# kausaltech/reina-model

Hardware: NVIDIA B200
Metric: agent-days/sec (HUS 1.7M) (higher is better)
Workload: dtype int32/f32 state, f64 uniforms

## Files before the change

### include/reina_b200.h

```cpp
#ifndef REINA_B200_H
#define REINA_B200_H

#include <stdint.h>

#ifdef __cplusplus
extern "C" {
#endif

#define RB_MAX_AGES 128
#define RB_MAX_VARIANTS 4
#define RB_MAX_ROWS 96
#define RB_NCDF 100
#define RB_MAX_IMPORT_EVENTS 8
#define RB_MAX_VACC 8
#define RB_MAX_IMPORT_CLASSES 16
#define RB_N_PLACES 6
#define RB_IOT_LEN 21

enum { RB_ASYMPTOMATIC = 0, RB_MILD, RB_SEVERE, RB_CRITICAL, RB_FATAL };
enum { RB_SUSCEPTIBLE = 0, RB_INCUBATION, RB_ILLNESS, RB_HOSPITALIZED, RB_IN_ICU, RB_RECOVERED, RB_DEAD };
enum { RB_NO_PROBLEMOS = 0, RB_TOO_MANY_INFECTEES, RB_TOO_MANY_CONTACTS, RB_HOSPITAL_ACCOUNTING_FAILURE,
       RB_NEGATIVE_CONTACTS, RB_MALLOC_FAILURE, RB_OTHER_FAILURE, RB_WRONG_STATE,
       RB_CONTACT_PROBABILITY_FAILURE, RB_INFECTEES_MISMATCH };
enum { RB_NO_TESTING = 0, RB_ALL_WITH_SYMPTOMS_CT, RB_ALL_WITH_SYMPTOMS, RB_ONLY_SEVERE_SYMPTOMS };
// ... 116 lines not shown
int rb_read_queue(rb_engine *e, int32_t replica, int32_t *out, int32_t cap, int32_t *n);
int rb_read_available(rb_engine *e, int32_t replica, int32_t *beds_icu);
float rb_last_step_ms(rb_engine *e);
#define RB_N_KERNELS 5
int rb_step_profiled(rb_engine *e, int32_t n_days, float *ms_per_kernel);
int rb_step_timed(rb_engine *e, int32_t n_days, float *ms_per_kernel, int32_t *launches_per_kernel, float *wall_ms);
int rb_comm_init(rb_engine *e, int32_t rank, int32_t nranks, const uint8_t *unique_id128);
int32_t rb_comm_rank(rb_engine *e);
int32_t rb_comm_size(rb_engine *e);
int rb_comm_allreduce(rb_engine *e, double *inout, int64_t n, int32_t op);
int rb_comm_allgather(rb_engine *e, const void *in, void *out, int64_t bytes_per_rank);
int rb_reduce_moments(rb_engine *e, int32_t day0, int32_t n, double *sum, double *sumsq, int64_t *n_replicas);

int rb_shard_unique_id(uint8_t *out128);
int rb_shard_init(rb_engine *e, int32_t rank, int32_t nranks, const uint8_t *unique_id128, float exchange_capacity);
int rb_shard_init_local(rb_engine **engines, int32_t nranks, float exchange_capacity);
int32_t rb_shard_rank(rb_engine *e);
int32_t rb_shard_nranks(rb_engine *e);
int64_t rb_shard_message_bytes(rb_engine *e);
int32_t rb_shard_exchange(rb_engine *e);

int64_t rb_state_bytes(rb_engine *e);
int rb_save_state(rb_engine *e, void *out, int64_t capacity);
int rb_load_state(rb_engine *e, const void *in, int64_t n_bytes);

int rb_branch(rb_engine *e, const int32_t *src, const uint32_t *seed);
int rb_read_seeds(rb_engine *e, uint32_t *out);

void rb_debug_flag(rb_engine *e, int32_t flag);
int rb_debug_phase_cycles(rb_engine *e, int32_t replica, long long *out16);

int64_t rb_launch_count(rb_engine *e);
int64_t rb_copied_bytes(rb_engine *e, int32_t direction);
const char *rb_last_error(void);

#ifdef __cplusplus
}
#endif
#endif
```

### reina_b200/_abi.py

```python
import ctypes as C
import os

import numpy as np

RB_MAX_AGES = 128
RB_MAX_VARIANTS = 4
RB_MAX_ROWS = 96
RB_NCDF = 100
RB_MAX_IMPORT_EVENTS = 8
RB_MAX_VACC = 8
RB_MAX_IMPORT_CLASSES = 16
RB_N_PLACES = 6
RB_IOT_LEN = 21
RB_N_TABLES = 6
RB_TX_BINS = 65
RB_PLACE_ROOT = RB_N_PLACES

ATTRS = ['susceptible', 'vaccinated', 'infected', 'all_infected', 'detected', 'all_detected',
         'in_icu', 'cum_icu', 'in_ward', 'dead', 'recovered', 'non_hospital_deaths', 'new_infections']
RB_N_ATTRS = len(ATTRS)
SCALARS = ['available_icu_units', 'available_hospital_beds', 'total_icu_units', 'total_hospital_beds',
           'total_infections', 'total_infectors', 'exposed_per_day', 'ct_cases_per_day', 'table_epoch',
           'day']
RB_S_CONTACTS0 = len(SCALARS)
# ... 32 lines not shown
    _fields_ = [
        ('testing_mode', C.c_int32), ('p_detected_anyway', C.c_float),
        ('p_successful_tracing', C.c_float), ('beds_delta', C.c_int32), ('icu_delta', C.c_int32),
        ('table_epoch', C.c_int32), ('n_imports', C.c_int32),
        ('import_amount', C.c_int32 * RB_MAX_IMPORT_EVENTS),
        ('import_variant', C.c_int32 * RB_MAX_IMPORT_EVENTS),
        ('trickle', C.c_int32 * RB_MAX_VARIANTS), ('n_vacc', C.c_int32),
        ('vacc_nr', C.c_int32 * RB_MAX_VACC), ('vacc_min_age', C.c_int32 * RB_MAX_VACC),
        ('vacc_max_age', C.c_int32 * RB_MAX_VACC), ('vacc_slot', C.c_int32 * RB_MAX_VACC),
        ('import_traced', C.c_int32), ('reserved', C.c_int32 * 3),
    ]


AGENT_DTYPE = np.dtype([
    ('infector', '<i4'), ('n_infected', '<i4'), ('days_left', '<i2'), ('day_of_illness', '<i2'),
    ('day_of_vaccination', '<i2'), ('state', 'u1'), ('severity', 'u1'), ('variant', 'u1'),
    ('flags', 'u1'), ('ward_days', 'u1'), ('icu_days', 'u1')], align=True)
assert AGENT_DTYPE.itemsize == 20, AGENT_DTYPE.itemsize

_HERE = os.path.dirname(os.path.abspath(__file__))
CUDA_LIB_PATH = os.environ.get('REINA_B200_LIB') or os.path.join(_HERE, 'libreina_b200.so')

SYMBOLS = ['create', 'destroy', 'reset', 'set_initial_state', 'step_profiled', 'set_contact_table', 'set_schedule', 'step', 'sync', 'day',
           'snapshot', 'row_len', 'read_stats', 'read_moments', 'read_per_age', 'problem', 'sample', 'read_agents',
           'read_queue', 'read_available', 'last_step_ms', 'launch_count', 'last_error', 'rng_block']


TX_SYMBOLS = ['transmission_len', 'transmission_stats', 'read_infection_days']
SX_SYMBOLS = ['transmission_settings_len', 'transmission_settings', 'read_infection_places']
BRANCH_SYMBOLS = ['branch', 'read_seeds']
SHARD_SYMBOLS = ['shard_unique_id', 'shard_init', 'shard_init_local', 'shard_rank', 'shard_nranks', 'shard_message_bytes', 'shard_exchange',
                 'state_bytes', 'save_state', 'load_state',
                 'comm_init', 'comm_rank', 'comm_size', 'comm_allreduce', 'comm_allgather', 'reduce_moments',
                 'step_timed', 'debug_flag', 'debug_phase_cycles', 'copied_bytes'] + TX_SYMBOLS + SX_SYMBOLS + BRANCH_SYMBOLS
SH_SHIFT = 12


def owner_of(agent_index, nranks):
    return (np.asarray(agent_index) >> SH_SHIFT) % nranks


class EngineError(RuntimeError):
    pass


def _ptr(a, ctype):
    return a.ctypes.data_as(C.POINTER(ctype))


class Library:

    def __init__(self, path, prefix):
        if not os.path.exists(path):
            raise EngineError(
                '%s not found: build it with `python -c "import __graft_entry__ as g; g.build()"` '
                '(there is no CPU fallback)' % path)
        self.path, self.prefix = path, prefix
        self.dll = C.CDLL(path)
        f = {}
        for name in SYMBOLS:
            f[name] = getattr(self.dll, prefix + name)
        vp = C.c_void_p
        f['create'].argtypes = [C.POINTER(Config), C.POINTER(C.c_int32), C.POINTER(C.c_int32),
                                C.POINTER(Variant), C.POINTER(C.c_int32), C.POINTER(C.c_int32),
                                C.POINTER(C.c_float), C.POINTER(vp)]
        f['destroy'].argtypes = [vp]
        f['destroy'].restype = None
# ... 24 lines not shown
        f['last_step_ms'].argtypes = [vp]
        f['last_step_ms'].restype = C.c_float
        f['launch_count'].argtypes = [vp]
        f['launch_count'].restype = C.c_int64
        f['last_error'].argtypes = []
        f['last_error'].restype = C.c_char_p
        if prefix == 'rb_':
            for name in SHARD_SYMBOLS:
                f[name] = getattr(self.dll, prefix + name)
            f['shard_unique_id'].argtypes = [C.c_char_p]
            f['shard_init'].argtypes = [vp, C.c_int32, C.c_int32, C.c_char_p, C.c_float]
            f['shard_init_local'].argtypes = [C.POINTER(vp), C.c_int32, C.c_float]
            f['shard_rank'].argtypes = [vp]
            f['shard_nranks'].argtypes = [vp]
            f['shard_message_bytes'].argtypes = [vp]
            f['shard_message_bytes'].restype = C.c_int64
            f['shard_exchange'].argtypes = [vp]
            f['state_bytes'].argtypes = [vp]
            f['state_bytes'].restype = C.c_int64
            f['save_state'].argtypes = [vp, C.c_void_p, C.c_int64]
            f['load_state'].argtypes = [vp, C.c_void_p, C.c_int64]
            f['comm_init'].argtypes = [vp, C.c_int32, C.c_int32, C.c_char_p]
            f['comm_rank'].argtypes = [vp]
            f['comm_size'].argtypes = [vp]
            f['comm_allreduce'].argtypes = [vp, C.POINTER(C.c_double), C.c_int64, C.c_int32]
            f['comm_allgather'].argtypes = [vp, C.c_void_p, C.c_void_p, C.c_int64]
            f['reduce_moments'].argtypes = [vp, C.c_int32, C.c_int32, C.POINTER(C.c_double), C.POINTER(C.c_double), C.POINTER(C.c_int64)]
            f['step_timed'].argtypes = [vp, C.c_int32, C.POINTER(C.c_float), C.POINTER(C.c_int32), C.POINTER(C.c_float)]
            f['debug_flag'].argtypes = [vp, C.c_int32]
            f['debug_flag'].restype = None
            f['debug_phase_cycles'].argtypes = [vp, C.c_int32, C.c_void_p]
            f['copied_bytes'].argtypes = [vp, C.c_int32]
            f['copied_bytes'].restype = C.c_int64
        self.f = f
        if prefix == 'rb_':
            self.bind_transmission()
            self.bind_settings()
            self.bind_branch()

    def bind_transmission(self):
        f, vp = self.f, C.c_void_p
        for name in TX_SYMBOLS:
            f[name] = getattr(self.dll, self.prefix + name)
        f['transmission_len'].argtypes = [vp]
        f['transmission_len'].restype = C.c_int32
        f['transmission_stats'].argtypes = [vp, C.POINTER(C.c_int32)]
        f['read_infection_days'].argtypes = [vp, C.c_int32, C.POINTER(C.c_int32)]

    def bind_settings(self):
        f, vp = self.f, C.c_void_p
        for name in SX_SYMBOLS:
            f[name] = getattr(self.dll, self.prefix + name)
        f['transmission_settings_len'].argtypes = [vp]
        f['transmission_settings_len'].restype = C.c_int32
        f['transmission_settings'].argtypes = [vp, C.POINTER(C.c_int32), C.c_int32, C.POINTER(C.c_int32)]
        f['read_infection_places'].argtypes = [vp, C.c_int32, C.POINTER(C.c_int32), C.c_int32, C.POINTER(C.c_int32)]

    def bind_branch(self):
        f, vp = self.f, C.c_void_p
        for name in BRANCH_SYMBOLS:
            f[name] = getattr(self.dll, self.prefix + name)
        f['branch'].argtypes = [vp, C.POINTER(C.c_int32), C.POINTER(C.c_uint32)]
        f['read_seeds'].argtypes = [vp, C.POINTER(C.c_uint32)]

    def check(self, rc, what):
        if rc != 0:
# ... 194 lines not shown
        out = np.empty((self.n_replicas, self.lib.f['transmission_settings_len'](self.h)), dtype=np.int32)
        self.lib.check(self.lib.f['transmission_settings'](self.h, _ptr(ep, C.c_int32), ep.size, _ptr(out, C.c_int32)),
                       'transmission_settings')
        return out

    def read_infection_places(self, replica, epoch_of_day):
        ep = np.ascontiguousarray(epoch_of_day, dtype=np.int32)
        out = np.empty(self.n_agents, dtype=np.int32)
        self.lib.check(self.lib.f['read_infection_places'](self.h, replica, _ptr(ep, C.c_int32), ep.size, _ptr(out, C.c_int32)),
                       'read_infection_places')
        return out

    def branch(self, src, seeds):
        s = np.ascontiguousarray(src, dtype=np.int32)
        k = np.ascontiguousarray(seeds, dtype=np.uint32)
        assert s.shape == k.shape == (self.n_replicas,)
        self.lib.check(self.lib.f['branch'](self.h, _ptr(s, C.c_int32), _ptr(k, C.c_uint32)), 'branch')

    def read_seeds(self):
        out = np.empty((self.n_replicas, self.cfg.max_days + 1), dtype=np.uint32)
        self.lib.check(self.lib.f['read_seeds'](self.h, _ptr(out, C.c_uint32)), 'read_seeds')
        return out

    def last_step_ms(self):
        return float(self.lib.f['last_step_ms'](self.h))

    def launch_count(self):
        return int(self.lib.f['launch_count'](self.h))

    def copied_bytes(self):
        f = self.lib.f['copied_bytes']
        return int(f(self.h, 0)), int(f(self.h, 1))


def shard_init_local(engines, exchange_capacity=0.0):
    lib = engines[0].lib
    arr = (C.c_void_p * len(engines))(*[e.h for e in engines])
    try:
        lib.check(lib.f['shard_init_local'](arr, len(engines), exchange_capacity), 'shard_init_local')
    except EngineError:
        for e in engines:
            e.half_joined = True
        raise
    for k, e in enumerate(engines):
        e.rank, e.nranks = k, len(engines)


def shard_unique_id(lib=None):
    lib = lib or cuda_library()
    buf = C.create_string_buffer(128)
    lib.check(lib.f['shard_unique_id'](buf), 'shard_unique_id')
    return buf.raw
```

### reina_b200/csrc/branch.cuh

```cuda
#ifndef REINA_B200_BRANCH_CUH
#define REINA_B200_BRANCH_CUH

#include "state.cuh"

__device__ __forceinline__ void branch_copy_bytes(void *dst, const void *src, size_t bytes, size_t tid, size_t nt) {
    if ((((uintptr_t)dst | (uintptr_t)src | bytes) & 15u) == 0) {
        uint4 *d = (uint4 *)dst; const uint4 *s = (const uint4 *)src;
        for (size_t i = tid; i < bytes / 16; i += nt) d[i] = s[i];
    } else {
        uint32_t *d = (uint32_t *)dst; const uint32_t *s = (const uint32_t *)src;
        for (size_t i = tid; i < bytes / 4; i += nt) d[i] = s[i];
    }
}

__global__ void k_branch_copy(Eng G, uint32_t *seed_of_day, const int32_t *src, const uint32_t *seed, int today) {
    const int j = blockIdx.y, s = src[j];
    const size_t tid = (size_t)blockIdx.x * blockDim.x + threadIdx.x, nt = (size_t)gridDim.x * blockDim.x;
    const size_t M = (size_t)G.max_days + 1;
    if (s != j) {
        const size_t N = G.Npad, W = G.sus_words, Q = 2 * (size_t)G.cap_queue, S = M * G.row_len;
        branch_copy_bytes(G.hot + j * N, G.hot + s * N, N * sizeof(uint32_t), tid, nt);
        branch_copy_bytes(G.rec + j * N, G.rec + s * N, N * sizeof(AgentRec), tid, nt);
        branch_copy_bytes(G.sus + j * W, G.sus + s * W, W * sizeof(uint32_t), tid, nt);
        branch_copy_bytes(G.det + j * W, G.det + s * W, W * sizeof(uint32_t), tid, nt);
        branch_copy_bytes(G.q_key + j * Q, G.q_key + s * Q, Q * sizeof(unsigned long long), tid, nt);
        branch_copy_bytes(G.q_agent + j * Q, G.q_agent + s * Q, Q * sizeof(int32_t), tid, nt);
        branch_copy_bytes(G.stats + j * S, G.stats + s * S, S * sizeof(int32_t), tid, nt);
        for (size_t i = tid; i < 2 * (size_t)G.n_seg; i += nt) G.seg_n[2 * (size_t)G.n_seg * j + i] = make_uint2(0u, 0u);
    }
    if (blockIdx.x != 0) return;
    const uint32_t *cs = reinterpret_cast<const uint32_t *>(&G.ctr[s]);
    uint32_t *cd = reinterpret_cast<uint32_t *>(&G.ctr[j]);
    const uint32_t seed_word = (uint32_t)(offsetof(RepCtr, seed) / 4);
    if (s != j)
        for (uint32_t w = threadIdx.x; w < (uint32_t)(sizeof(RepCtr) / 4); w += blockDim.x) cd[w] = w == seed_word ? seed[j] : cs[w];
    else if (threadIdx.x == 0) cd[seed_word] = seed[j];
    const uint32_t *hs = seed_of_day + (size_t)s * M;
    uint32_t *hd = seed_of_day + (size_t)j * M;
    for (size_t d = threadIdx.x; d < M; d += blockDim.x)
        if ((int)d >= today) hd[d] = seed[j]; else if (s != j) hd[d] = hs[d];
}

__global__ void k_branch_rebuild(Eng G, const int32_t *src) {
    const int r = blockIdx.y;
    if (src[r] == r) return;
    RepCtr *c = &G.ctr[r];
    const size_t base = (size_t)r * G.Npad;
    const uint32_t cur = c->lsel;
    for (int a = blockIdx.x * blockDim.x + threadIdx.x; a < G.N; a += gridDim.x * blockDim.x) {
        uint32_t h = G.hot[base + a];
        const uint32_t st = H_STATE(h);
        if (st == RB_SUSCEPTIBLE) continue;
        G.perm[base + a] = sweep_slot(G, c, (uint32_t)a);
        if (!((st >= RB_INCUBATION && st <= RB_IN_ICU) || (st >= RB_RECOVERED && !(h & H_INCL)))) continue;
        if (h & H_QUEUED) h |= H_DET;
        list_add(G, r, c, cur, (uint32_t)a, h);
    }
}

__global__ void k_init_seeds(Eng G, uint32_t *seed_of_day, uint32_t seed, int from_ctr) {
    const int r = blockIdx.x;
// ... 6 lines not shown
```

### reina_b200/csrc/engine.cu

```cuda
#include "state.cuh"
#include "boundary.cuh"
#include "sweep.cuh"
#include "contacts.cuh"
#include "shard.cuh"
#include "setup.cuh"
#include "run.cuh"
#include "transmission.cuh"
#include "branch.cuh"

static thread_local char g_err[512];
#define CK(call) do { cudaError_t e_ = (call); if (e_ != cudaSuccess) { snprintf(g_err, sizeof g_err, "%s:%d %s: %s", __FILE__, __LINE__, #call, cudaGetErrorString(e_)); return 1; } } while (0)

#define MAX_GROUPS 8
struct ReplicaGroup {
    int r0, R;
    int sweep_blocks, list_blocks, resolve_blocks;
    cudaStream_t stream;
    cudaEvent_t ev_stagger, ev_join;
    cudaGraphExec_t graph[2];
};

struct rb_engine {
    rb_config cfg;
    Eng G;
// ... 173 lines not shown
    float cc = cfg->contact_capacity > 0 ? cfg->contact_capacity : 1.0f;
    G.cap_items = pow2_at_least((uint64_t)((double)N * cc) + 4096);
    G.cap_succ = pow2_at_least((uint64_t)N / 8 + 4096);
    G.cap_events = pow2_at_least((uint64_t)N / 16 + 2048);
    G.cap_queue = pow2_at_least((uint64_t)N / 8 + 2048);
    const size_t RN = (size_t)R * G.Npad;
    cudaDeviceProp prop; CK(cudaGetDeviceProperties(&prop, cfg->device));
    const int sms = prop.multiProcessorCount;
    e->run_ctas = 0; e->run_boundary_ctas = 1;
    {
        int per_sm = 0;
        CK(cudaOccupancyMaxActiveBlocksPerMultiprocessor(&per_sm, k_run, RUN_THREADS, 0));
        const long long total = (long long)per_sm * sms;
        bool on = false;
        if (const char *s = getenv("RB_PERSISTENT")) on = atoi(s) != 0;
        if (on && total >= 2LL * R) {
            long long t = total / R; if (t > 64) t = 64;
            if (const char *s = getenv("RB_RUN_CTAS")) { const int v = atoi(s); if (v >= 1 && (long long)v * R <= total) t = v; }
            e->run_ctas = (int)t;
            int b = 1; while (b * 2 <= t && b * 2 <= 16) b *= 2;
            e->run_boundary_ctas = b;
        }
    }
    {
        int ng, pct;
        group_config(R, &ng, &pct);
        long long ctas = (long long)sms * SW_CTAS_PER_SM * (ng > 1 ? pct : 100) / 100 / ((R + ng - 1) / ng);
        if (ctas < 1) ctas = 1;
        long long S = 2 * ctas * SW_WARPS, most = (long long)N / 256;
        if (e->run_ctas) S = 2LL * e->run_ctas * RUN_WARPS;
        if (S > most) S = most;
        G.n_seg = (uint32_t)(S < 1 ? 1 : S);
        G.seg_cap = ((uint32_t)N + G.n_seg - 1) / G.n_seg;
    }
    G.sus_words = ((G.Npad + 31) / 32 + 32 + 3) & ~3;
    if (dalloc(e, &G.hot, RN) || dalloc(e, &G.perm, RN) || dalloc(e, &G.rec, RN) ||
        dalloc(e, &G.sus, (size_t)R * G.sus_words) || dalloc(e, &G.det, (size_t)R * G.sus_words) || dalloc(e, &G.alist, (size_t)R * 2 * G.n_seg * G.seg_cap) || dalloc(e, &G.seg_n, (size_t)R * 2 * G.n_seg) || dalloc(e, &G.items, (size_t)R * G.cap_items) || dalloc(e, &G.succ, (size_t)R * G.cap_succ) ||
        dalloc(e, &G.ev_key, (size_t)R * G.cap_events) || dalloc(e, &G.ev_agent, (size_t)R * G.cap_events) ||
        dalloc(e, &G.q_key, (size_t)R * 2 * G.cap_queue) || dalloc(e, &G.q_agent, (size_t)R * 2 * G.cap_queue) ||
        dalloc(e, &G.ctr, (size_t)R) || dalloc(e, &G.stats, (size_t)R * (cfg->max_days + 1) * G.row_len) ||
        dalloc(e, &e->seed_of_day, (size_t)R * (cfg->max_days + 1)) ||
        dalloc(e, &e->d_sched, (size_t)cfg->max_days + 1) ||
        dalloc(e, &e->d_moments, 2 * ((size_t)cfg->max_days + 1) * G.row_len + 2)) { rb_destroy(e); return 1; }
    G.sched = e->d_sched;
    e->h_sched.assign(cfg->max_days + 1, rb_day_params());
    e->n_table_slots = 1024;
    if (dalloc(e, &e->d_tables, (size_t)e->n_table_slots)) { rb_destroy(e); return 1; }
    CK(cudaMemset(e->d_tables, 0, sizeof(DevTable *) * e->n_table_slots));
    G.tables = e->d_tables;
    e->tables.assign(e->n_table_slots, nullptr);
    rb_variant *dv; int32_t *d_as, *d_ga, *d_ilo, *d_ihi; float *d_icum; uint8_t *d_ab;
    if (dalloc(e, &dv, (size_t)cfg->n_variants) || dalloc(e, &d_as, (size_t)cfg->n_ages + 1) || dalloc(e, &d_ga, (size_t)cfg->n_ages) ||
        dalloc(e, &d_ilo, (size_t)RB_MAX_IMPORT_CLASSES) || dalloc(e, &d_ihi, (size_t)RB_MAX_IMPORT_CLASSES) ||
        dalloc(e, &d_icum, (size_t)RB_MAX_IMPORT_CLASSES) || dalloc(e, &d_ab, (size_t)(G.Npad >> 10) + 2)) { rb_destroy(e); return 1; }
    {
        std::vector<uint8_t> ab((size_t)(G.Npad >> 10) + 2);
        int age = 0;
        for (size_t b = 0; b < ab.size(); b++) {
            int64_t a = (int64_t)b << 10; if (a > N - 1) a = N - 1;
            while (age < cfg->n_ages - 1 && e->age_start[age + 1] <= a) age++;
            ab[b] = (uint8_t)age;
        }
        CK(cudaMemcpy(d_ab, ab.data(), ab.size(), cudaMemcpyHostToDevice));
    }
    e->h_variants.assign(variants, variants + cfg->n_variants);
    CK(cudaMemcpy(dv, variants, sizeof(rb_variant) * cfg->n_variants, cudaMemcpyHostToDevice));
    CK(cudaMemcpy(d_as, e->age_start.data(), sizeof(int32_t) * (cfg->n_ages + 1), cudaMemcpyHostToDevice));
    CK(cudaMemcpy(d_ga, group_of_age, sizeof(int32_t) * cfg->n_ages, cudaMemcpyHostToDevice));
    CK(cudaMemcpy(d_ilo, import_lo, sizeof(int32_t) * cfg->n_import_classes, cudaMemcpyHostToDevice));
    CK(cudaMemcpy(d_ihi, import_hi, sizeof(int32_t) * cfg->n_import_classes, cudaMemcpyHostToDevice));
// ... 700 lines not shown
extern "C" int rb_sync(rb_engine *e) {
    CK(cudaSetDevice(e->cfg.device));
    CK(cudaStreamSynchronize(e->stream));
    float ms = 0;
    if (cudaEventElapsedTime(&ms, e->ev0, e->ev1) == cudaSuccess) e->last_ms = ms; else cudaGetLastError();
    if (!e->shard_events.empty()) {
        double t[6] = {0, 0, 0, 0, 0, 0};
        for (size_t d = 0; d + 7 <= e->shard_events.size(); d += 7)
            for (int k = 0; k < 6; k++) { float x = 0; if (cudaEventElapsedTime(&x, e->shard_events[d + k], e->shard_events[d + k + 1]) == cudaSuccess) t[k] += x; }
        fprintf(stderr, "[rank %d] %zu days: sweep %.2f  expose %.2f  exchange+wait %.2f  merge %.2f  resolve %.2f  boundary %.2f ms (step %.2f)\n",
                e->G.rank, e->shard_events.size() / 7, t[0], t[1], t[2], t[3], t[4], t[5], e->last_ms);
        for (cudaEvent_t ev : e->shard_events) cudaEventDestroy(ev);
        e->shard_events.clear();
    }
    return 0;
}

extern "C" int32_t rb_day(rb_engine *e) { return e->day; }
extern "C" void rb_debug_flag(rb_engine *e, int32_t v) { e->G.dbg = v; }
extern "C" int rb_debug_phase_cycles(rb_engine *e, int32_t replica, long long *out16) {
    cudaSetDevice(e->cfg.device); cudaStreamSynchronize(e->stream);
    RepCtr c; if (cudaMemcpy(&c, &e->G.ctr[replica], sizeof c, cudaMemcpyDeviceToHost) != cudaSuccess) return 1;
    memcpy(out16, c.dbg_t, sizeof c.dbg_t); return 0;
}
extern "C" int rb_rng_block(int32_t words, uint32_t key, const uint32_t *ctr, uint32_t *out) {
    if (words == 4) { const u32x4 x = philox(key, ctr[0], ctr[1], ctr[2], ctr[3]); out[0] = x.x; out[1] = x.y; out[2] = x.z; out[3] = x.w; return 0; }
    snprintf(g_err, sizeof g_err, "rb_rng_block: words must be 4");
    return 1;
}
extern "C" int32_t rb_row_len(rb_engine *e) { return e->G.row_len; }
extern "C" float rb_last_step_ms(rb_engine *e) { return e->last_ms; }
extern "C" int64_t rb_launch_count(rb_engine *e) { return e->launches; }
extern "C" int64_t rb_copied_bytes(rb_engine *e, int32_t direction) { return direction == 0 ? e->h2d_bytes : e->d2h_bytes; }

extern "C" int rb_snapshot(rb_engine *e) {
    CK(cudaSetDevice(e->cfg.device));
    k_snapshot<<<e->G.R, 256, 0, e->stream>>>(e->G); e->launches++;
    CK(cudaGetLastError());
    return 0;
}

extern "C" int rb_read_stats(rb_engine *e, int32_t day0, int32_t n, int32_t *out) {
    CK(cudaSetDevice(e->cfg.device));
    if (day0 < 0 || day0 + n > e->cfg.max_days + 1) { snprintf(g_err, sizeof g_err, "stats range"); return 1; }
    const Eng &G = e->G;
    CK(cudaMemcpy2DAsync(out, sizeof(int32_t) * (size_t)n * G.row_len,
                         G.stats + (size_t)day0 * G.row_len, sizeof(int32_t) * (size_t)(G.max_days + 1) * G.row_len,
                         sizeof(int32_t) * (size_t)n * G.row_len, G.R, cudaMemcpyDeviceToHost, e->stream));
    CK(cudaStreamSynchronize(e->stream));
    e->d2h_bytes += (int64_t)sizeof(int32_t) * n * G.row_len * G.R;
    return 0;
}

extern "C" int rb_read_moments(rb_engine *e, int32_t day0, int32_t n, double *sum, double *sumsq) {
    CK(cudaSetDevice(e->cfg.device));
    if (day0 < 0 || n < 1 || day0 + n > e->cfg.max_days + 1) { snprintf(g_err, sizeof g_err, "stats range"); return 1; }
    const size_t cnt = (size_t)n * e->G.row_len;
    double *d = e->d_moments;
    k_moments<<<n, 160, 0, e->stream>>>(e->G, day0, d, d + cnt); e->launches++;
    CK(cudaGetLastError());
    CK(cudaMemcpyAsync(sum, d, sizeof(double) * cnt, cudaMemcpyDeviceToHost, e->stream));
    CK(cudaMemcpyAsync(sumsq, d + cnt, sizeof(double) * cnt, cudaMemcpyDeviceToHost, e->stream));
    CK(cudaStreamSynchronize(e->stream));
    e->d2h_bytes += (int64_t)sizeof(double) * 2 * cnt;
    return 0;
}
// ... 301 lines not shown
```

### reina_b200/csrc/state.cuh

```cuda
#ifndef REINA_B200_STATE_CUH
#define REINA_B200_STATE_CUH

#include <cuda_runtime.h>
#include <stdint.h>
#include <stdio.h>
#include <string.h>

#include <dlfcn.h>
#include <nccl.h>

#include <algorithm>
#include <vector>

#include "../../include/reina_b200.h"
#include "rng.cuh"

#define MAX_INFECTEES 64
#define MAX_CONTACTS 128

#define H_STATE(h) ((h) & 7u)
#define H_SEV(h) (((h) >> 3) & 7u)
#define H_DET (1u << 6)
#define H_QUEUED (1u << 7)
#define H_VAR(h) (((h) >> 8) & 3u)
// ... 75 lines not shown
    alignas(128) uint32_t n_succ;
    alignas(128) int32_t exposed_per_day;
    int32_t total_infectors, total_infections;
    alignas(128) uint32_t n_events;
    uint32_t n_newq;
    uint32_t n_upd;
    alignas(128) int32_t daily_contacts[RB_N_PLACES];
    int32_t by_variant[RB_MAX_VARIANTS];
    alignas(128) int32_t drain_det[RB_MAX_AGES];
    alignas(128) uint32_t n_l0;
    uint32_t n_l1, n_edges;
    alignas(128) unsigned int run_bar;
    unsigned int run_exit;
    alignas(128) unsigned int wide_bar;
    alignas(128) uint32_t wide_day;
    int32_t wide_mp[WIDE_MAX_CTAS][4];
    long long dbg_t[16];
    long long dbg_last;
};

struct Eng {
    int32_t dbg;
    int32_t N, Npad, n_ages, n_groups, n_variants, R, max_days, row_len, n_import_classes, fhalf;
    uint32_t cap_items, cap_succ, cap_events, cap_queue;
    uint32_t *hot;
    uint32_t *perm;
    AgentRec *rec;
    uint32_t *sus;
    int32_t sus_words;
    uint32_t *det;
    uint2 *alist;
    uint2 *seg_n;
    uint32_t n_seg, seg_cap;
    uint2 *items;
    Attempt *succ;
    unsigned long long *ev_key; int32_t *ev_agent;
    unsigned long long *q_key; int32_t *q_agent;
    RepCtr *ctr;
    int32_t *stats;
    const rb_day_params *sched;
    DevTable *const *tables;
    const rb_variant *variants;
    const int32_t *age_start;
    const uint8_t *age_blk;
    const int32_t *group_of_age;
    const int32_t *import_lo, *import_hi; const float *import_cum;
    int32_t rank, nranks;
    int32_t wide_min;
    int32_t r0;
    uint8_t *xbuf; size_t xslot;
    uint8_t *xpeer[MAX_RANKS];
    int32_t xp2p; const uint32_t *xepoch;
    uint32_t xcap_q, xcap_ev, xcap_upd, xcap_succ;
};

#define XFLAG_BYTES 256
#define SH_SHIFT 12
__device__ __forceinline__ uint32_t xflag_value(const Eng &G, int day) { return *G.xepoch * 65536u + (uint32_t)day + 1u; }
__device__ __forceinline__ bool owns(const Eng &G, uint32_t a) { return G.nranks == 1 || (int)((a >> SH_SHIFT) % (uint32_t)G.nranks) == G.rank; }

struct XSlot {
    RepCtr *hdr;
    unsigned long long *q_key; int32_t *q_agent;
    unsigned long long *ev_key; int32_t *ev_agent;
    uint2 *upd;
    struct Attempt *succ;
// ... 32 lines not shown
    const uint32_t s = G.perm[(size_t)r * G.Npad + a];
    return s >= c->start ? s - c->start : s + (uint32_t)G.N - c->start;
}
__device__ __forceinline__ void mark_detected(const Eng &G, int r, int32_t a) {
    atomicOr(&G.det[(size_t)r * G.sus_words + (a >> 5)], 1u << (a & 31));
}
__device__ __forceinline__ void count_add(RepCtr *c, int attr, int age, int d) { atomicAdd(&c->counts[attr][age], d); }
__device__ __forceinline__ void set_problem(RepCtr *c, int p) { atomicCAS(&c->problem, 0, p); }

__device__ __forceinline__ int symptom_severity(const rb_variant *v, int age, float val, bool vacc_eff) {
    float vmod = 1.0f;
    if (vacc_eff) vmod = vmod * 0.1f;
    float syc = v->tab[RB_T_SYMPTOMATIC][age];
    if (val >= syc) return RB_ASYMPTOMATIC;
    syc = syc * vmod;
    float dohc = v->tab[RB_T_DEATH_OUTSIDE_HOSPITAL][age];
    if (dohc != 0.0f) {
        if (val < dohc * syc) return RB_FATAL;
        val = (val - dohc) / (1.0f - dohc);
    }
    float sc = v->tab[RB_T_SEVERE][age], cc = v->tab[RB_T_CRITICAL][age], fc = v->tab[RB_T_FATAL][age];
    if (val < ((fc * cc) * sc) * syc) return RB_FATAL;
    if (val < (cc * sc) * syc) return RB_CRITICAL;
    if (val < sc * syc) return RB_SEVERE;
    return RB_MILD;
}

__device__ __forceinline__ uint2 *seg_ptr(const Eng &G, int r, uint32_t which, uint32_t s) {
    return G.alist + (((size_t)r * 2 + which) * G.n_seg + s) * G.seg_cap;
}
__device__ __forceinline__ uint2 *seg_count(const Eng &G, int r, uint32_t which, uint32_t s) {
    return G.seg_n + ((size_t)r * 2 + which) * G.n_seg + s;
}
__device__ __forceinline__ void list_add(const Eng &G, int r, RepCtr *c, uint32_t which, uint32_t a, uint32_t w) {
    const uint32_t s = a % G.n_seg;
    const uint32_t k = atomicAdd(&seg_count(G, r, which, s)->y, 1u);
    if (k < G.seg_cap) seg_ptr(G, r, which, s)[G.seg_cap - 1u - k] = make_uint2(a, w); else set_problem(c, RB_OTHER_FAILURE);
}

__device__ void device_infect(const Eng &G, int r, RepCtr *c, int32_t t, int32_t src, uint32_t src_h, int variant,
                              int slot, bool fresh, int list, bool has_list) {
    const size_t base = (size_t)r * G.Npad;
    const int day = c->day;
    uint32_t old = 0; int32_t prev_child = -1;
    if (src >= 0) {
        old = atomicAdd(&G.rec[base + src].cold, 1u);
        prev_child = atomicExch(&G.rec[base + src].first_child, t);
    }
    const int vd = c->any_vacc ? (int)G.rec[base + t].vacc_day : -1;
    const int age = age_of(G, t);
    const rb_variant *v0 = &G.variants[0];
    const bool vacc_eff = vd >= 0 && (day - vd) > 14;
    int sev = 0, dl = 0;
    if (owns(G, (uint32_t)t)) {
        u32x4 x = philox(c->seed, (uint32_t)t, (uint32_t)day, PU_SEVERITY, 0);
        sev = symptom_severity(v0, age, u01f(x.x), vacc_eff);
        dl = clamp255(round_to_int(gamma_f(c->seed, (uint32_t)t, (uint32_t)day, PU_INCUB, v0->incubation_kappa, v0->incubation_theta)));
    }
    if (src >= 0) {
        variant = (int)H_VAR(src_h);
        G.rec[base + t].infector = src;
        if ((src_h & H_LIST) && (old & 0xffffu) >= MAX_INFECTEES) set_problem(c, RB_TOO_MANY_INFECTEES);
        G.rec[base + t].inf_key = ((uint32_t)day << 8) | (uint32_t)slot;
        G.rec[base + t].next_sib = prev_child;
    } else {
        G.rec[base + t].inf_key = (uint32_t)day << 8;
// ... 21 lines not shown
```

### reina_b200/csrc/sweep.cuh

```cuda
#ifndef REINA_B200_SWEEP_CUH
#define REINA_B200_SWEEP_CUH
#include "state.cuh"

#ifndef SW_THREADS
#define SW_THREADS 128
#endif
#define SW_WARPS (SW_THREADS / 32)
#define SW_RCAP 64
#ifndef SW_CTAS_PER_SM
#define SW_CTAS_PER_SM 9
#endif

struct WarpRings {
    uint32_t ea[SW_RCAP], ed[SW_RCAP];
    uint32_t ta[SW_RCAP], tw[SW_RCAP];
};

__device__ __forceinline__ uint32_t ring_push(uint32_t *ra, uint32_t *rb, uint32_t tail, bool want, uint32_t x, uint32_t y, int lane) {
    const uint32_t m = __ballot_sync(0xffffffffu, want);
    if (want) { uint32_t p = (tail + __popc(m & ((1u << lane) - 1u))) & (SW_RCAP - 1); ra[p] = x; rb[p] = y; }
    return tail + __popc(m);
}

__device__ __forceinline__ void seg_append(const Eng &G, RepCtr *c, uint2 *out, uint32_t &out_n, bool want, uint32_t a, uint32_t w, int lane) {
    const uint32_t m = __ballot_sync(0xffffffffu, want);
    if (want) {
        const uint32_t p = out_n + __popc(m & ((1u << lane) - 1u));
        if (p < G.seg_cap) out[p] = make_uint2(a, w); else set_problem(c, RB_OTHER_FAILURE);
    }
    out_n += __popc(m);
}

struct SweepOut {
    RepCtr *cd;
    unsigned long long *q_key; int32_t *q_agent; uint32_t cap_q;
    unsigned long long *ev_key; int32_t *ev_agent; uint32_t cap_ev;
    uint2 *upd; uint32_t cap_upd;
};
__device__ __forceinline__ SweepOut sweep_out(const Eng &G, int r, RepCtr *c) {
    SweepOut O;
    if (!G.xbuf) {
        const size_t qb = ((size_t)r * 2 + (c->qsel ^ 1u)) * G.cap_queue;
        O.cd = c; O.q_key = G.q_key + qb; O.q_agent = G.q_agent + qb; O.cap_q = G.cap_queue;
        O.ev_key = G.ev_key + (size_t)r * G.cap_events; O.ev_agent = G.ev_agent + (size_t)r * G.cap_events; O.cap_ev = G.cap_events;
        O.upd = nullptr; O.cap_upd = 0;
    } else {
        const XSlot x = xslot_of(G, G.rank, c->day);
        O.cd = x.hdr; O.q_key = x.q_key; O.q_agent = x.q_agent; O.cap_q = G.xcap_q;
// ... 158 lines not shown
    if (keep) list_add(G, r, cd, next, a, lw);
    if (O.upd) {
        const uint32_t mk = __ballot_sync(0xffffffffu, changed);
        uint32_t b = 0;
        if (lane == 0 && mk) b = atomicAdd(&O.cd->n_upd, (uint32_t)__popc(mk));
        b = __shfl_sync(0xffffffffu, b, 0);
        if (changed) {
            const uint32_t idx = b + __popc(mk & ((1u << lane) - 1u));
            if (idx < O.cap_upd) O.upd[idx] = make_uint2(a, h); else set_problem(O.cd, RB_OTHER_FAILURE);
        }
    }
}

__device__ __forceinline__ void stage_entry(const Eng &G, uint32_t &w, bool &keep, bool &want_e, bool &want_t, uint32_t &desc) {
    const uint32_t st = H_STATE(w);
    if ((w & H_PEND) || st >= RB_RECOVERED) { want_t = true; return; }
    if (w & H_FRESH) { w &= ~H_FRESH; keep = true; return; }
    const uint32_t sev = H_SEV(w), var = H_VAR(w);
    uint32_t dl = H_DL(w);
    if (st == RB_INCUBATION || st == RB_ILLNESS) {
        const int dayidx = st == RB_INCUBATION ? -(int)dl : (int)H_DOI(w);
        if (!(w & H_DET) && dayidx >= -10 && dayidx <= 10 && G.variants[var].iot[dayidx + 10] != 0.0f) {
            want_e = true;
            const uint32_t cls = (st == RB_ILLNESS && sev != RB_ASYMPTOMATIC) ? 1u : 0u;
            desc = ((uint32_t)(dayidx + 10) << 14) | ((sev == RB_ASYMPTOMATIC ? 1u : 0u) << 19) | (var << 20) | (cls << 22);
        }
        if (st == RB_ILLNESS) { uint32_t doi = H_DOI(w); if (doi < 31) doi++; w = H_SET_DOI(w, doi); }
    }
    if (dl > 0) dl--;
    w = H_SET_DL(w, dl);
    if (dl == 0) want_t = true; else keep = true;
}

__device__ __forceinline__ void sweep_warp(const Eng &G, const int r, const uint32_t first, const uint32_t n_warps, WarpRings &W, const int lane) {
    RepCtr *c = &G.ctr[r];
    const DevTable *tb = G.tables[c->epoch];
    uint2 *items = G.items + (size_t)r * G.cap_items;
    RepCtr *cd = !G.xbuf ? c : xslot_of(G, G.rank, c->day).hdr;
    const uint32_t cur = c->lsel;
    uint32_t e_head = 0, e_tail = 0, t_head = 0, t_tail = 0;

    uint2 cnt_next = make_uint2(0u, 0u);
    if (first < G.n_seg) cnt_next = *seg_count(G, r, cur, first);
    for (uint32_t seg = first; ; seg += n_warps) {
        const bool tail = seg >= G.n_seg;
        const uint2 cnt = cnt_next;
        cnt_next = make_uint2(0u, 0u);
        if (seg + n_warps < G.n_seg) cnt_next = *seg_count(G, r, cur, seg + n_warps);
        const uint32_t nf = min(cnt.x, G.seg_cap), n = min(cnt.x + cnt.y, G.seg_cap);
        const uint2 *in = seg_ptr(G, r, cur, tail ? 0u : seg);
        uint2 *out = seg_ptr(G, r, cur ^ 1u, tail ? 0u : seg);
        uint32_t out_n = 0;
        const uint32_t gap = G.seg_cap - n;
        auto entry = [&](uint32_t i) { return __ldcs(&in[i < nf ? i : i + gap]); };
        uint2 ent = make_uint2(0u, 0u);
        if ((uint32_t)lane < n) ent = entry(lane);
        uint32_t i0 = 0;
        bool again;
        do {
            if (i0 < n) {
                const bool valid = i0 + lane < n;
                const uint2 cur_ent = ent;
                if (i0 + 32 + lane < n) ent = entry(i0 + 32 + lane);
                bool keep = false, want_e = false, want_t = false;
                uint32_t w = cur_ent.y, desc = 0;
                if (valid) stage_entry(G, w, keep, want_e, want_t, desc);
                seg_append(G, cd, out, out_n, keep, cur_ent.x, w, lane);
                e_tail = ring_push(W.ea, W.ed, e_tail, want_e, cur_ent.x, desc, lane);
                t_tail = ring_push(W.ta, W.tw, t_tail, want_t, cur_ent.x, w, lane);
                __syncwarp();
            }
            const uint32_t e_av = e_tail - e_head, t_av = t_tail - t_head;
            if (e_av >= 32 || (tail && e_av)) { const uint32_t m = min(32u, e_av); stage_expose(G, r, c, cd, tb, W, e_head, m, items, lane); e_head += m; }
            if (t_av >= 32 || (tail && t_av)) { const uint32_t m = min(32u, t_av); stage_slow(G, r, c, cd, W, t_head, m, cur ^ 1u, lane); t_head += m; }
            __syncwarp();
            i0 += 32;
            again = tail ? (e_tail != e_head || t_tail != t_head) : i0 < n;
        } while (again);
        if (tail) break;
        if (lane == 0) seg_count(G, r, cur ^ 1u, seg)->x = out_n;
    }
}
__global__ void __launch_bounds__(SW_THREADS, SW_CTAS_PER_SM) k_sweep(Eng G) {
    __shared__ WarpRings s_rings[SW_WARPS];
    const int warp = threadIdx.x >> 5;
    sweep_warp(G, blockIdx.y + G.r0, blockIdx.x * SW_WARPS + warp, gridDim.x * SW_WARPS, s_rings[warp], threadIdx.x & 31);
}

__global__ void k_flush_lists(Eng G) {
    const int r = blockIdx.y;
    const RepCtr *c = &G.ctr[r];
    const size_t base = (size_t)r * G.Npad;
    const uint32_t cur = c->lsel;
    const int lane = threadIdx.x & 31;
    const uint32_t n_warps = gridDim.x * (blockDim.x >> 5);
    for (uint32_t seg = blockIdx.x * (blockDim.x >> 5) + (threadIdx.x >> 5); seg < G.n_seg; seg += n_warps) {
        const uint2 cnt = *seg_count(G, r, cur, seg);
        const uint32_t nf = min(cnt.x, G.seg_cap), n = min(cnt.x + cnt.y, G.seg_cap);
        const uint2 *in = seg_ptr(G, r, cur, seg);
        for (uint32_t i = lane; i < n; i += 32) {
            const uint2 e = in[i < nf ? i : i + (G.seg_cap - n)];
            if ((e.y & H_PEND) || H_STATE(e.y) >= RB_RECOVERED) continue;
            const uint32_t h = G.hot[base + e.x];
            G.hot[base + e.x] = (h & ~(H_DAYS_MASK | H_FRESH)) | (e.y & (H_DAYS_MASK | H_FRESH));
        }
    }
}
__global__ void k_rebuild_lists(Eng G) {
    const int r = blockIdx.y;
    RepCtr *c = &G.ctr[r];
    const size_t base = (size_t)r * G.Npad;
    const uint32_t cur = c->lsel;
    for (int a = blockIdx.x * blockDim.x + threadIdx.x; a < G.N; a += gridDim.x * blockDim.x) {
        if (!owns(G, (uint32_t)a)) continue;
        uint32_t h = G.hot[base + a];
        const uint32_t st = H_STATE(h);
        if (!((st >= RB_INCUBATION && st <= RB_IN_ICU) || (st >= RB_RECOVERED && !(h & H_INCL)))) continue;
        if (h & H_QUEUED) h |= H_DET;
        G.perm[base + a] = sweep_slot(G, c, (uint32_t)a);
        list_add(G, r, c, cur, (uint32_t)a, h);
    }
}
__global__ void k_clear_lists(Eng G) {
    const size_t n = (size_t)G.R * 2 * G.n_seg;
    for (size_t i = (size_t)blockIdx.x * blockDim.x + threadIdx.x; i < n; i += (size_t)gridDim.x * blockDim.x) G.seg_n[i] = make_uint2(0u, 0u);
}

#endif
```

Before: 744.9 billion.

## Park long-idle active agents in per-segment day buckets to skip daily sweeps

Adds a per-segment timing wheel of 64 day buckets. Agents whose next transition is several days away (hospitalized, in ICU, detected, or long ill) are moved out of the active list into the bucket for their wake-up day. Each day the sweep only reads the bucket for that day, fast-forwards those agents' counters, and sends them to the slow transition stage. This is meant to cut the per-day cost of re-reading and re-writing stable active entries. In exchange it adds bucket bookkeeping, shared-memory atomics, extra memory, and flush and clear paths, plus overflow handling when a bucket is full.

Result: faster. 762.0 billion, median of 6 (+2.3%).

```diff
diff --git a/include/reina_b200.h b/include/reina_b200.h
--- a/include/reina_b200.h
+++ b/include/reina_b200.h
@@ -172,6 +172,7 @@
 
 int64_t rb_launch_count(rb_engine *e);
 int64_t rb_copied_bytes(rb_engine *e, int32_t direction);
+int rb_park_stats(rb_engine *e, int64_t *out4);
 const char *rb_last_error(void);
 
 #ifdef __cplusplus
diff --git a/reina_b200/_abi.py b/reina_b200/_abi.py
--- a/reina_b200/_abi.py
+++ b/reina_b200/_abi.py
@@ -88,7 +88,7 @@
 SHARD_SYMBOLS = ['shard_unique_id', 'shard_init', 'shard_init_local', 'shard_rank', 'shard_nranks', 'shard_message_bytes', 'shard_exchange',
                  'state_bytes', 'save_state', 'load_state',
                  'comm_init', 'comm_rank', 'comm_size', 'comm_allreduce', 'comm_allgather', 'reduce_moments',
-                 'step_timed', 'debug_flag', 'debug_phase_cycles', 'copied_bytes'] + TX_SYMBOLS + SX_SYMBOLS + BRANCH_SYMBOLS
+                 'step_timed', 'debug_flag', 'debug_phase_cycles', 'copied_bytes', 'park_stats'] + TX_SYMBOLS + SX_SYMBOLS + BRANCH_SYMBOLS
 SH_SHIFT = 12
 
 
@@ -179,6 +179,7 @@
             f['debug_phase_cycles'].argtypes = [vp, C.c_int32, C.c_void_p]
             f['copied_bytes'].argtypes = [vp, C.c_int32]
             f['copied_bytes'].restype = C.c_int64
+            f['park_stats'].argtypes = [vp, C.POINTER(C.c_int64)]
         self.f = f
         if prefix == 'rb_':
             self.bind_transmission()
@@ -439,6 +440,11 @@
         f = self.lib.f['copied_bytes']
         return int(f(self.h, 0)), int(f(self.h, 1))
 
+    def park_stats(self):
+        out = np.zeros(4, dtype=np.int64)
+        self.lib.check(self.lib.f['park_stats'](self.h, _ptr(out, C.c_int64)), 'park_stats')
+        return {'woken': int(out[0]), 'full': int(out[1]), 'parked': int(out[2]), 'fullest_bucket': int(out[3])}
+
 
 def shard_init_local(engines, exchange_capacity=0.0):
     lib = engines[0].lib
diff --git a/reina_b200/csrc/branch.cuh b/reina_b200/csrc/branch.cuh
--- a/reina_b200/csrc/branch.cuh
+++ b/reina_b200/csrc/branch.cuh
@@ -27,6 +27,7 @@
         branch_copy_bytes(G.q_agent + j * Q, G.q_agent + s * Q, Q * sizeof(int32_t), tid, nt);
         branch_copy_bytes(G.stats + j * S, G.stats + s * S, S * sizeof(int32_t), tid, nt);
         for (size_t i = tid; i < 2 * (size_t)G.n_seg; i += nt) G.seg_n[2 * (size_t)G.n_seg * j + i] = make_uint2(0u, 0u);
+        for (size_t i = tid; i < (size_t)G.n_seg * PARK_B; i += nt) G.park_n[(size_t)G.n_seg * PARK_B * j + i] = 0u;
     }
     if (blockIdx.x != 0) return;
     const uint32_t *cs = reinterpret_cast<const uint32_t *>(&G.ctr[s]);
diff --git a/reina_b200/csrc/engine.cu b/reina_b200/csrc/engine.cu
--- a/reina_b200/csrc/engine.cu
+++ b/reina_b200/csrc/engine.cu
@@ -229,10 +229,16 @@
         if (S > most) S = most;
         G.n_seg = (uint32_t)(S < 1 ? 1 : S);
         G.seg_cap = ((uint32_t)N + G.n_seg - 1) / G.n_seg;
+#ifdef PARK_CAP
+        G.park_cap = PARK_CAP;
+#else
+        G.park_cap = std::max(32u, G.seg_cap / 32);
+#endif
     }
     G.sus_words = ((G.Npad + 31) / 32 + 32 + 3) & ~3;
     if (dalloc(e, &G.hot, RN) || dalloc(e, &G.perm, RN) || dalloc(e, &G.rec, RN) ||
-        dalloc(e, &G.sus, (size_t)R * G.sus_words) || dalloc(e, &G.det, (size_t)R * G.sus_words) || dalloc(e, &G.alist, (size_t)R * 2 * G.n_seg * G.seg_cap) || dalloc(e, &G.seg_n, (size_t)R * 2 * G.n_seg) || dalloc(e, &G.items, (size_t)R * G.cap_items) || dalloc(e, &G.succ, (size_t)R * G.cap_succ) ||
+        dalloc(e, &G.sus, (size_t)R * G.sus_words) || dalloc(e, &G.det, (size_t)R * G.sus_words) || dalloc(e, &G.alist, (size_t)R * 2 * G.n_seg * G.seg_cap) || dalloc(e, &G.seg_n, (size_t)R * 2 * G.n_seg) ||
+        dalloc(e, &G.park, (size_t)R * G.n_seg * PARK_B * G.park_cap) || dalloc(e, &G.park_n, (size_t)R * G.n_seg * PARK_B) || dalloc(e, &G.park_stat, (size_t)R * G.n_seg) || dalloc(e, &G.items, (size_t)R * G.cap_items) || dalloc(e, &G.succ, (size_t)R * G.cap_succ) ||
         dalloc(e, &G.ev_key, (size_t)R * G.cap_events) || dalloc(e, &G.ev_agent, (size_t)R * G.cap_events) ||
         dalloc(e, &G.q_key, (size_t)R * 2 * G.cap_queue) || dalloc(e, &G.q_agent, (size_t)R * 2 * G.cap_queue) ||
         dalloc(e, &G.ctr, (size_t)R) || dalloc(e, &G.stats, (size_t)R * (cfg->max_days + 1) * G.row_len) ||
@@ -999,6 +1005,19 @@
 extern "C" float rb_last_step_ms(rb_engine *e) { return e->last_ms; }
 extern "C" int64_t rb_launch_count(rb_engine *e) { return e->launches; }
 extern "C" int64_t rb_copied_bytes(rb_engine *e, int32_t direction) { return direction == 0 ? e->h2d_bytes : e->d2h_bytes; }
+extern "C" int rb_park_stats(rb_engine *e, int64_t *out) {
+    CK(cudaSetDevice(e->cfg.device));
+    const Eng &G = e->G;
+    std::vector<uint2> st((size_t)G.R * G.n_seg);
+    std::vector<uint32_t> pn((size_t)G.R * G.n_seg * PARK_B);
+    CK(cudaMemcpyAsync(st.data(), G.park_stat, st.size() * sizeof(st[0]), cudaMemcpyDeviceToHost, e->stream));
+    CK(cudaMemcpyAsync(pn.data(), G.park_n, pn.size() * sizeof(pn[0]), cudaMemcpyDeviceToHost, e->stream));
+    CK(cudaStreamSynchronize(e->stream));
+    out[0] = out[1] = out[2] = out[3] = 0;
+    for (const uint2 &x : st) { out[0] += x.x; out[1] += x.y; }
+    for (uint32_t n : pn) { out[2] += std::min(n, G.park_cap); out[3] = std::max<int64_t>(out[3], std::min(n, G.park_cap)); }
+    return 0;
+}
 
 extern "C" int rb_snapshot(rb_engine *e) {
     CK(cudaSetDevice(e->cfg.device));
diff --git a/reina_b200/csrc/state.cuh b/reina_b200/csrc/state.cuh
--- a/reina_b200/csrc/state.cuh
+++ b/reina_b200/csrc/state.cuh
@@ -131,6 +131,10 @@
     uint2 *alist;
     uint2 *seg_n;
     uint32_t n_seg, seg_cap;
+    uint2 *park;
+    uint32_t *park_n;
+    uint2 *park_stat;
+    uint32_t park_cap;
     uint2 *items;
     Attempt *succ;
     unsigned long long *ev_key; int32_t *ev_agent;
@@ -229,6 +233,13 @@
 __device__ __forceinline__ uint2 *seg_count(const Eng &G, int r, uint32_t which, uint32_t s) {
     return G.seg_n + ((size_t)r * 2 + which) * G.n_seg + s;
 }
+#define PARK_B 64
+__device__ __forceinline__ uint2 *park_ptr(const Eng &G, int r, uint32_t s, uint32_t b) {
+    return G.park + (((size_t)r * G.n_seg + s) * PARK_B + b) * G.park_cap;
+}
+__device__ __forceinline__ uint32_t *park_count(const Eng &G, int r, uint32_t s) {
+    return G.park_n + ((size_t)r * G.n_seg + s) * PARK_B;
+}
 __device__ __forceinline__ void list_add(const Eng &G, int r, RepCtr *c, uint32_t which, uint32_t a, uint32_t w) {
     const uint32_t s = a % G.n_seg;
     const uint32_t k = atomicAdd(&seg_count(G, r, which, s)->y, 1u);
diff --git a/reina_b200/csrc/sweep.cuh b/reina_b200/csrc/sweep.cuh
--- a/reina_b200/csrc/sweep.cuh
+++ b/reina_b200/csrc/sweep.cuh
@@ -14,6 +14,8 @@
 struct WarpRings {
     uint32_t ea[SW_RCAP], ed[SW_RCAP];
     uint32_t ta[SW_RCAP], tw[SW_RCAP];
+    uint32_t pn[PARK_B];
+    uint2 ps;
 };
 
 __device__ __forceinline__ uint32_t ring_push(uint32_t *ra, uint32_t *rb, uint32_t tail, bool want, uint32_t x, uint32_t y, int lane) {
@@ -238,40 +240,72 @@
     if (dl == 0) want_t = true; else keep = true;
 }
 
+#ifndef PARK_MIN_DL
+#define PARK_MIN_DL 1
+#endif
+__device__ __forceinline__ bool parkable(uint32_t w) {
+    const uint32_t st = H_STATE(w);
+    return H_DL(w) >= PARK_MIN_DL && H_DL(w) < PARK_B && (st == RB_HOSPITALIZED || st == RB_IN_ICU || (w & H_DET) || (st == RB_ILLNESS && H_DOI(w) > 10));
+}
+__device__ __forceinline__ uint32_t park_advance(uint32_t w, uint32_t k) {
+    if (H_STATE(w) == RB_ILLNESS) w = H_SET_DOI(w, min(31u, H_DOI(w) + k));
+    return H_SET_DL(w, H_DL(w) - k);
+}
+
 __device__ __forceinline__ void sweep_warp(const Eng &G, const int r, const uint32_t first, const uint32_t n_warps, WarpRings &W, const int lane) {
     RepCtr *c = &G.ctr[r];
     const DevTable *tb = G.tables[c->epoch];
     uint2 *items = G.items + (size_t)r * G.cap_items;
     RepCtr *cd = !G.xbuf ? c : xslot_of(G, G.rank, c->day).hdr;
     const uint32_t cur = c->lsel;
+    const uint32_t today = (uint32_t)c->day & (PARK_B - 1);
     uint32_t e_head = 0, e_tail = 0, t_head = 0, t_tail = 0;
 
     uint2 cnt_next = make_uint2(0u, 0u);
-    if (first < G.n_seg) cnt_next = *seg_count(G, r, cur, first);
+    uint32_t nb_next = 0;
+    if (first < G.n_seg) { cnt_next = *seg_count(G, r, cur, first); nb_next = park_count(G, r, first)[today]; }
     for (uint32_t seg = first; ; seg += n_warps) {
         const bool tail = seg >= G.n_seg;
         const uint2 cnt = cnt_next;
-        cnt_next = make_uint2(0u, 0u);
-        if (seg + n_warps < G.n_seg) cnt_next = *seg_count(G, r, cur, seg + n_warps);
+        const uint32_t nb = nb_next;
+        cnt_next = make_uint2(0u, 0u); nb_next = 0;
+        if (seg + n_warps < G.n_seg) { cnt_next = *seg_count(G, r, cur, seg + n_warps); nb_next = park_count(G, r, seg + n_warps)[today]; }
         const uint32_t nf = min(cnt.x, G.seg_cap), n = min(cnt.x + cnt.y, G.seg_cap);
         const uint2 *in = seg_ptr(G, r, cur, tail ? 0u : seg);
         uint2 *out = seg_ptr(G, r, cur ^ 1u, tail ? 0u : seg);
         uint32_t out_n = 0;
+        const uint32_t nt = n + nb;
         const uint32_t gap = G.seg_cap - n;
-        auto entry = [&](uint32_t i) { return __ldcs(&in[i < nf ? i : i + gap]); };
+        auto entry = [&](uint32_t i) { return __ldcs(i < n ? &in[i < nf ? i : i + gap] : &park_ptr(G, r, seg, today)[i - n]); };
         uint2 ent = make_uint2(0u, 0u);
-        if ((uint32_t)lane < n) ent = entry(lane);
+        if ((uint32_t)lane < nt) ent = entry(lane);
+        if (!tail) {
+            const uint32_t *pc = park_count(G, r, seg);
+            W.pn[lane] = lane == (int)today ? 0u : pc[lane];
+            W.pn[lane + 32] = lane + 32 == (int)today ? 0u : pc[lane + 32];
+            if (lane == 0) W.ps = G.park_stat[(size_t)r * G.n_seg + seg];
+            __syncwarp();
+        }
         uint32_t i0 = 0;
         bool again;
         do {
-            if (i0 < n) {
-                const bool valid = i0 + lane < n;
+            if (i0 < nt) {
+                const bool valid = i0 + lane < nt;
                 const uint2 cur_ent = ent;
-                if (i0 + 32 + lane < n) ent = entry(i0 + 32 + lane);
+                if (i0 + 32 + lane < nt) ent = entry(i0 + 32 + lane);
                 bool keep = false, want_e = false, want_t = false;
                 uint32_t w = cur_ent.y, desc = 0;
-                if (valid) stage_entry(G, w, keep, want_e, want_t, desc);
-                seg_append(G, cd, out, out_n, keep, cur_ent.x, w, lane);
+                if (valid) {
+                    if (i0 + lane < n) stage_entry(G, w, keep, want_e, want_t, desc);
+                    else { w = park_advance(w, H_DL(w)); want_t = true; }
+                }
+                bool park = keep && !(cur_ent.y & H_FRESH) && parkable(w);
+                if (park) {
+                    const uint32_t b = (today + H_DL(w)) & (PARK_B - 1);
+                    const uint32_t k = atomicAdd(&W.pn[b], 1u);
+                    if (k < G.park_cap) park_ptr(G, r, seg, b)[k] = make_uint2(cur_ent.x, w); else park = false;
+                }
+                seg_append(G, cd, out, out_n, keep && !park, cur_ent.x, w, lane);
                 e_tail = ring_push(W.ea, W.ed, e_tail, want_e, cur_ent.x, desc, lane);
                 t_tail = ring_push(W.ta, W.tw, t_tail, want_t, cur_ent.x, w, lane);
                 __syncwarp();
@@ -281,10 +315,18 @@
             if (t_av >= 32 || (tail && t_av)) { const uint32_t m = min(32u, t_av); stage_slow(G, r, c, cd, W, t_head, m, cur ^ 1u, lane); t_head += m; }
             __syncwarp();
             i0 += 32;
-            again = tail ? (e_tail != e_head || t_tail != t_head) : i0 < n;
+            again = tail ? (e_tail != e_head || t_tail != t_head) : i0 < nt;
         } while (again);
         if (tail) break;
         if (lane == 0) seg_count(G, r, cur ^ 1u, seg)->x = out_n;
+        uint32_t *pc = park_count(G, r, seg);
+        const uint32_t p0 = W.pn[lane], p1 = W.pn[lane + 32];
+        pc[lane] = min(p0, G.park_cap); pc[lane + 32] = min(p1, G.park_cap);
+        uint32_t full = (p0 - min(p0, G.park_cap)) + (p1 - min(p1, G.park_cap));
+#pragma unroll
+        for (int o = 16; o > 0; o >>= 1) full += __shfl_xor_sync(0xffffffffu, full, o);
+        if (lane == 0) G.park_stat[(size_t)r * G.n_seg + seg] = make_uint2(W.ps.x + nb, W.ps.y + full);
+        __syncwarp();
     }
 }
 __global__ void __launch_bounds__(SW_THREADS, SW_CTAS_PER_SM) k_sweep(Eng G) {
@@ -310,6 +352,18 @@
             const uint32_t h = G.hot[base + e.x];
             G.hot[base + e.x] = (h & ~(H_DAYS_MASK | H_FRESH)) | (e.y & (H_DAYS_MASK | H_FRESH));
         }
+        const uint32_t *pc = park_count(G, r, seg);
+        for (uint32_t b = 0; b < PARK_B; b++) {
+            const uint32_t m = min(pc[b], G.park_cap);
+            const uint32_t dl = ((b - (uint32_t)c->day) & (PARK_B - 1)) + 1;
+            const uint2 *bk = park_ptr(G, r, seg, b);
+            for (uint32_t i = lane; i < m; i += 32) {
+                const uint2 e = bk[i];
+                const uint32_t w = park_advance(e.y, H_DL(e.y) - dl);
+                const uint32_t h = G.hot[base + e.x];
+                G.hot[base + e.x] = (h & ~(H_DAYS_MASK | H_FRESH)) | (w & H_DAYS_MASK);
+            }
+        }
     }
 }
 __global__ void k_rebuild_lists(Eng G) {
@@ -328,8 +382,10 @@
     }
 }
 __global__ void k_clear_lists(Eng G) {
-    const size_t n = (size_t)G.R * 2 * G.n_seg;
+    const size_t n = (size_t)G.R * 2 * G.n_seg, np = (size_t)G.R * G.n_seg * PARK_B;
     for (size_t i = (size_t)blockIdx.x * blockDim.x + threadIdx.x; i < n; i += (size_t)gridDim.x * blockDim.x) G.seg_n[i] = make_uint2(0u, 0u);
+    for (size_t i = (size_t)blockIdx.x * blockDim.x + threadIdx.x; i < np; i += (size_t)gridDim.x * blockDim.x) G.park_n[i] = 0u;
+    for (size_t i = (size_t)blockIdx.x * blockDim.x + threadIdx.x; i < (size_t)G.R * G.n_seg; i += (size_t)gridDim.x * blockDim.x) G.park_stat[i] = make_uint2(0u, 0u);
 }
 
 #endif
```
